# rohanpsingh/LearningHumanoidWalking

Hardware: AMD Instinct MI355X
Metric: env-steps/s (whole job): on-device rollout + GAE + PPO update (higher is better)
Workload: dtype f64 physics / f32 networks

## Files before the change

learninghumanoidwalking_amd/csrc/lhw_learner.h:

```cpp
#pragma once
#include "lhw_internal.h"

struct LearnerCore {
  int device = 0, D = 0, Dp = 0, A = 0, H = 0, learn_std = 0;
  float clip, ent_coeff, mirror_coeff, grad_clip, lr, adam_eps, beta1, beta2;
  int use_mirror = 0;
  size_t off_actor = 0, off_std = 0, off_critic = 0, n_critic = 0, n_params = 0;
  int *d_obs_src = nullptr, *d_act_src = nullptr;
  float *d_obs_sign = nullptr, *d_act_sign = nullptr;
  float *stats = nullptr;
  float *stats_part = nullptr;
  float *norm_part = nullptr;
  LhwDevMem mem;
};
#define SUMSQ_BLOCKS 128

int learner_check(const LhwPpoConfig* c, void** out, bool caps_ok);
void learner_init(LearnerCore& k, const LhwPpoConfig* c, size_t n_actor, size_t n_critic);
bool learner_mirror(LearnerCore& k, const LhwPpoConfig* c);
int learner_normalize(LearnerCore* k, const float* obs, int64_t R, const float* obs_mean, const float* obs_std, float* xn, float* xm, void* stream);
int learner_apply(LearnerCore* k, float* theta, float* grad, float* adam_m, float* adam_v, int64_t step, float grad_scale, void* stream);
int learner_grad_sqnorms(LearnerCore* k, float* out2_host);

struct AdamArgs {
  float *theta, *grad, *m, *v;
  size_t n0, off1, n1;
  int blocks0;
  float gscale;
  float* part;
  float* normsq_out;
  float max_norm, lr, beta1, beta2, eps, bc1, bc2sqrt;
};
AdamArgs learner_adam_args(const LearnerCore& k, float* theta, float* grad, float* adam_m, float* adam_v, int64_t step, float grad_scale);
__global__ void adam2_kernel(AdamArgs a);

struct StreamPair {
  hipStream_t s, sc;
  hipEvent_t ev_fork, ev_join;
  void fork() const { if (sc != s) { (void)hipEventRecord(ev_fork, s); (void)hipStreamWaitEvent(sc, ev_fork, 0); } }
  void join() const { if (sc != s) { (void)hipEventRecord(ev_join, sc); (void)hipStreamWaitEvent(s, ev_join, 0); } }
};

__global__ void normalize_kernel(const float* __restrict__ obs, int D, int Dp, size_t R, const float* __restrict__ mean, const float* __restrict__ stdv,
                                 float* __restrict__ xn, float* __restrict__ xm, const int* __restrict__ src, const float* __restrict__ sign);
__global__ void sample_kernel(const float* __restrict__ mu, int ldmu, int A, int N, const float* __restrict__ stdv, uint64_t seed, uint32_t env_base,
                              uint32_t counter, int deterministic, float* __restrict__ act, float* __restrict__ logp);
__global__ void ppo_loss_kernel(int B, int Rcap, int A, int Op, const float* __restrict__ ya, const float* __restrict__ yc, const float* __restrict__ act,
                                const float* __restrict__ old_logp, const float* __restrict__ adv, const float* __restrict__ ret,
                                const float* __restrict__ stdv, float clip, float mirror_coeff, int use_mirror, const int* __restrict__ act_src,
                                const float* __restrict__ act_sign, float* __restrict__ dya, float* __restrict__ dyc, float* __restrict__ dstd,
                                float* __restrict__ stats_part, const float* __restrict__ imit_target, const unsigned char* __restrict__ imit_mask,
                                float imit_coeff, float imit_inv_count, int seqB, float gscale);
__global__ void ppo_stats_rows_kernel(int B, int A, const float* __restrict__ rows, int ld, float imit_inv_count, float* __restrict__ stats_part);
__global__ void reduce_rows_kernel(const float* __restrict__ part, int nrows, int n, float* __restrict__ out);
__global__ void entropy_grad_kernel(const float* __restrict__ stdv, int A, float ent_coeff, float* __restrict__ grad_std);
```

learninghumanoidwalking_amd/csrc/lhw_learner.hip:

```cpp
#include "lhw_learner.h"

#include <cmath>
#include <mutex>
#include <vector>

#include "lhw_policy.h"
#include "lhw_rng.h"

__global__ void normalize_kernel(const float* __restrict__ obs, int D, int Dp, size_t R, const float* __restrict__ mean,
                                 const float* __restrict__ stdv, float* __restrict__ xn, float* __restrict__ xm,
                                 const int* __restrict__ src, const float* __restrict__ sign) {
  size_t i = (size_t)blockIdx.x * blockDim.x + threadIdx.x;
  if (i >= R * (size_t)Dp) return;
  size_t r = i / Dp;
  int j = (int)(i - r * Dp);
  float v = 0.f, vm = 0.f;
  if (j < D) {
    v = (obs[r * D + j] - mean[j]) / stdv[j];
    if (xm) vm = (sign[j] * obs[r * D + src[j]] - mean[j]) / stdv[j];
  }
  xn[i] = v;
  if (xm) xm[i] = vm;
}
__global__ void __launch_bounds__(256) sample_kernel(const float* __restrict__ mu, int ldmu, int A, int N, const float* __restrict__ stdv,
                                                     uint64_t seed, uint32_t env_base, uint32_t counter, int deterministic,
                                                     float* __restrict__ act, float* __restrict__ logp) {
  __shared__ float terms[8][32];
  LHW_LDS_POISON(terms);
  const int r = threadIdx.x >> 5, a = threadIdx.x & 31, n = blockIdx.x * 8 + r;
  if (n < N && a < A) {
    float term;
    act[(size_t)n * A + a] = lhw_policy_sample(mu[(size_t)n * ldmu + a], stdv[a], seed, env_base + n, counter, a, deterministic, &term);
    terms[r][a] = term;
  }
  __syncthreads();
  if (n < N && a == 0) {
    float lp = 0.f;
    for (int k = 0; k < A; k++) lp += terms[r][k];
    logp[n] = lp;
  }
}
__device__ __forceinline__ void ppo_stats_block(float (&vals)[NSTAT], float* __restrict__ stats_part) {
  __shared__ float red[NSTAT][4];
  LHW_LDS_POISON(red);
  for (int o = 32; o > 0; o >>= 1)
    for (int k = 0; k < NSTAT; k++) vals[k] += __shfl_xor(vals[k], o);
  int lane = threadIdx.x & 63, wave = threadIdx.x >> 6;
  if (lane == 0)
    for (int k = 0; k < NSTAT; k++) red[k][wave] = vals[k];
  __syncthreads();
  if (threadIdx.x < NSTAT) stats_part[(size_t)blockIdx.x * NSTAT + threadIdx.x] = (red[threadIdx.x][0] + red[threadIdx.x][1]) + (red[threadIdx.x][2] + red[threadIdx.x][3]);
}
__global__ void __launch_bounds__(256) ppo_loss_kernel(int B, int Rcap, int A, int Op, const float* __restrict__ ya,
                                                       const float* __restrict__ yc, const float* __restrict__ act,
                                                       const float* __restrict__ old_logp, const float* __restrict__ adv,
                                                       const float* __restrict__ ret, const float* __restrict__ stdv,
                                                       float clip, float mirror_coeff, int use_mirror,
                                                       const int* __restrict__ act_src, const float* __restrict__ act_sign,
                                                       float* __restrict__ dya, float* __restrict__ dyc,
                                                       float* __restrict__ dstd , float* __restrict__ stats_part,
                                                       const float* __restrict__ imit_target ,
                                                       const unsigned char* __restrict__ imit_mask , float imit_coeff,
                                                       float imit_inv_count, int seqB,
                                                       float gscale ) {
  int m = blockIdx.x * blockDim.x + threadIdx.x;
  size_t rn = (size_t)m, rm = (size_t)Rcap + m;
  if (seqB > 0 && use_mirror) { rn = (size_t)(m / seqB) * (2 * (size_t)seqB) + (size_t)(m % seqB); rm = rn + seqB; }
  const LhwPpoHead h{B, A, Op, act, old_logp, adv, ret, stdv, clip, mirror_coeff, use_mirror, act_src, act_sign, dstd, imit_target, imit_mask,
                     imit_coeff, imit_inv_count, gscale};
  float t[NSTAT] = {0, 0, 0, 0, 0, 0};
  const float invB = 1.f / (float)B, invBA = 1.f / ((float)B * (float)A);
  if (m < B) {
    lhw_ppo_actor_row(h, m, ya + rn * Op, ya + rm * Op, dya + rn * Op, dya + rm * Op, 1, t);
    float dv;
    t[1] = lhw_ppo_critic_row(h, m, yc[(size_t)m * 4], &dv);
    dyc[(size_t)m * 4] = dv;
    dyc[(size_t)m * 4 + 1] = 0.f; dyc[(size_t)m * 4 + 2] = 0.f; dyc[(size_t)m * 4 + 3] = 0.f;
  }
  float vals[NSTAT] = {t[0] * invB, t[1] * invB, t[2] * invBA, t[3] * invB, t[4] * invB, t[5] * imit_inv_count};
  ppo_stats_block(vals, stats_part);
}

__global__ void __launch_bounds__(256) ppo_stats_rows_kernel(int B, int A, const float* __restrict__ rows, int ld, float imit_inv_count,
                                                             float* __restrict__ stats_part) {
  const int m = blockIdx.x * blockDim.x + threadIdx.x;
  float t[NSTAT] = {0, 0, 0, 0, 0, 0};
  if (m < B)
    for (int k = 0; k < NSTAT; k++) t[k] = rows[(size_t)k * ld + m];
  const float invB = 1.f / (float)B, invBA = 1.f / ((float)B * (float)A);
  float vals[NSTAT] = {t[0] * invB, t[1] * invB, t[2] * invBA, t[3] * invB, t[4] * invB, t[5] * imit_inv_count};
  ppo_stats_block(vals, stats_part);
}

__global__ void reduce_rows_kernel(const float* __restrict__ part, int nrows, int n, float* __restrict__ out) {
  int k = threadIdx.x;
  if (k >= n) return;
  float s = 0.f;
  for (int b = 0; b < nrows; b++) s += part[(size_t)b * n + k];
  out[k] += s;
}

__global__ void entropy_grad_kernel(const float* __restrict__ stdv, int A, float ent_coeff, float* __restrict__ grad_std) {
  int a = threadIdx.x;
  if (a < A) grad_std[a] += -ent_coeff / ((float)A * stdv[a]);
}
__global__ void __launch_bounds__(256) sumsq2_kernel(const float* __restrict__ g0, size_t n0, const float* __restrict__ g1, size_t n1, float scale,
                                                     float* __restrict__ part ) {
  const int grp = blockIdx.x / SUMSQ_BLOCKS, b = blockIdx.x - grp * SUMSQ_BLOCKS;
  const float* __restrict__ g = grp ? g1 : g0;
  const size_t n = grp ? n1 : n0;
  float s = 0.f;
  for (size_t i = (size_t)b * blockDim.x + threadIdx.x; i < n; i += (size_t)SUMSQ_BLOCKS * blockDim.x) {
    float v = g[i] * scale;
    s += v * v;
  }
  for (int o = 32; o > 0; o >>= 1) s += __shfl_xor(s, o);
  __shared__ float red[4];
  LHW_LDS_POISON(red);
  if ((threadIdx.x & 63) == 0) red[threadIdx.x >> 6] = s;
  __syncthreads();
  if (threadIdx.x == 0) part[blockIdx.x] = (red[0] + red[1]) + (red[2] + red[3]);
}
__global__ void __launch_bounds__(256) adam2_kernel(AdamArgs a) {
  float *__restrict__ theta = a.theta, *__restrict__ grad = a.grad, *__restrict__ m = a.m, *__restrict__ v = a.v, *__restrict__ normsq_out = a.normsq_out;
  const float* __restrict__ part = a.part;
  const size_t n0 = a.n0, off1 = a.off1, n1 = a.n1;
  const int blocks0 = a.blocks0;
  const float gscale = a.gscale, max_norm = a.max_norm, lr = a.lr, beta1 = a.beta1, beta2 = a.beta2, eps = a.eps, bc1 = a.bc1, bc2sqrt = a.bc2sqrt;
  const int grp = (int)blockIdx.x >= blocks0 ? 1 : 0;
  __shared__ float nsq;
  LHW_LDS_POISON(nsq);
  if (threadIdx.x == 0) {
    float s = 0.f;
    for (int b = 0; b < SUMSQ_BLOCKS; b++) s += part[grp * SUMSQ_BLOCKS + b];
    nsq = s;
    if ((int)blockIdx.x == (grp ? blocks0 : 0)) normsq_out[grp] = s;
  }
  __syncthreads();
  const size_t i = (size_t)((int)blockIdx.x - (grp ? blocks0 : 0)) * blockDim.x + threadIdx.x;
  if (i >= (grp ? n1 : n0)) return;
  const size_t e = (grp ? off1 : 0) + i;
  float norm = sqrtf(nsq);
  float coef = max_norm / (norm + 1e-6f);
  coef = coef < 1.f ? coef : 1.f;
  float g = grad[e] * gscale * coef;
  float mi = beta1 * m[e] + (1.f - beta1) * g;
  float vi = beta2 * v[e] + (1.f - beta2) * g * g;
  m[e] = mi; v[e] = vi;
  float denom = sqrtf(vi) / bc2sqrt + eps;
  theta[e] -= (lr / bc1) * (mi / denom);
  grad[e] = 0.f;
}
__global__ void __launch_bounds__(256) gae_kernel(int T, int N, const float* __restrict__ rew, const float* __restrict__ val,
                                                  const uint8_t* __restrict__ done, const float* __restrict__ vterm,
                                                  const float* __restrict__ vfinal, double gamma, double lam,
                                                  float* __restrict__ ret, float* __restrict__ adv) {
  int n = blockIdx.x * blockDim.x + threadIdx.x;
  if (n >= N) return;
  double gae = 0.0, nextv = (double)vfinal[n];
  for (int t = T - 1; t >= 0; t--) {
    size_t i = (size_t)t * N + n;
    uint8_t f = done[i];
    if (f) {
      nextv = (f & 1) ? 0.0 : (double)vterm[i];
      gae = 0.0;
    }
    double v = (double)val[i];
    double delta = (double)rew[i] + gamma * nextv - v;
    gae = delta + gamma * lam * gae;
    double r = gae + v;
    ret[i] = (float)r;
    adv[i] = (float)r - val[i];
    nextv = v;
  }
}

#define MOM_BLOCKS 256
__global__ void __launch_bounds__(256) moments_kernel(const float* __restrict__ x, size_t n, double* __restrict__ part) {
  double s = 0, s2 = 0;
  for (size_t i = (size_t)blockIdx.x * blockDim.x + threadIdx.x; i < n; i += (size_t)gridDim.x * blockDim.x) {
    double v = x[i];
    s += v; s2 += v * v;
  }
  for (int o = 32; o > 0; o >>= 1) { s += __shfl_xor(s, o); s2 += __shfl_xor(s2, o); }
  __shared__ double red[2][4];
  LHW_LDS_POISON(red);
  if ((threadIdx.x & 63) == 0) { red[0][threadIdx.x >> 6] = s; red[1][threadIdx.x >> 6] = s2; }
  __syncthreads();
  if (threadIdx.x == 0) {
    part[2 * blockIdx.x] = (red[0][0] + red[0][1]) + (red[0][2] + red[0][3]);
    part[2 * blockIdx.x + 1] = (red[1][0] + red[1][1]) + (red[1][2] + red[1][3]);
  }
}
__global__ void moments_final_kernel(const double* __restrict__ part, int n, double* __restrict__ out) {
  if (threadIdx.x < 2) {
    double s = 0;
    for (int b = 0; b < n; b++) s += part[2 * b + threadIdx.x];
    out[threadIdx.x] = s;
  }
}
__global__ void scale_shift_kernel(float* __restrict__ x, size_t n, float mean, float inv) {
  size_t i = (size_t)blockIdx.x * blockDim.x + threadIdx.x;
  if (i < n) x[i] = (x[i] - mean) * inv;
}

__global__ void standardize_kernel(float* __restrict__ x, size_t n, const double* __restrict__ st, double eps) {
  const double cnt = st[2], mean = st[0] / cnt;
  const double var = fmax(0.0, (st[1] - cnt * mean * mean) / fmax(1.0, cnt - 1.0));
  const float mean_f = (float)mean, inv_f = (float)(1.0 / (sqrt(var) + eps));
  size_t i = (size_t)blockIdx.x * blockDim.x + threadIdx.x;
  if (i < n) x[i] = (x[i] - mean_f) * inv_f;
}
// ... 14 lines not shown
  k.use_mirror = c->mirror_obs_src != nullptr;
  k.off_actor = 0; k.off_std = n_actor; k.off_critic = k.off_std + pad4(k.A); k.n_critic = n_critic; k.n_params = k.off_critic + n_critic;
}
bool learner_mirror(LearnerCore& k, const LhwPpoConfig* c) {
  if (!k.use_mirror) return true;
  std::vector<int> osrc(k.Dp, 0), asrc(k.A, 0);
  std::vector<float> osgn(k.Dp, 0.f), asgn(k.A, 0.f);
  for (int j = 0; j < k.D; j++) { osrc[j] = c->mirror_obs_src[j]; osgn[j] = c->mirror_obs_sign[j]; if (osrc[j] < 0 || osrc[j] >= k.D) return false; }
  for (int j = 0; j < k.A; j++) { asrc[j] = c->mirror_act_src[j]; asgn[j] = c->mirror_act_sign[j]; if (asrc[j] < 0 || asrc[j] >= k.A) return false; }
  k.d_obs_src = k.mem.put(osrc.data(), osrc.size()); k.d_act_src = k.mem.put(asrc.data(), asrc.size());
  k.d_obs_sign = k.mem.put(osgn.data(), osgn.size()); k.d_act_sign = k.mem.put(asgn.data(), asgn.size());
  return !k.mem.failed();
}
int learner_normalize(LearnerCore* k, const float* obs, int64_t R, const float* obs_mean, const float* obs_std, float* xn, float* xm,
                             void* stream) {
  if (!k || !obs || !xn || R <= 0) return lhw_fail(LHW_ERR_ARG, "bad argument");
  if (xm && !k->use_mirror) return lhw_fail(LHW_ERR_ARG, "mirror output requested but no mirror tables configured");
  HIPCHK(hipSetDevice(k->device));
  size_t n = (size_t)R * k->Dp;
  hipLaunchKernelGGL(normalize_kernel, dim3((n + 255) / 256), dim3(256), 0, (hipStream_t)stream, obs, k->D, k->Dp, (size_t)R,
                     obs_mean, obs_std, xn, xm, k->d_obs_src, k->d_obs_sign);
  HIPCHK(hipGetLastError());
  return LHW_OK;
}
#define LHW_MAX_DEVICES 64
static int device_of(const void* ptr, int* dev) {
  hipPointerAttribute_t at;
  if (hipPointerGetAttributes(&at, ptr) != hipSuccess) return lhw_fail(LHW_ERR_ARG, "not a device pointer");
  if (at.device < 0 || at.device >= LHW_MAX_DEVICES) return lhw_fail(LHW_ERR_ARG, "device %d out of range", at.device);
  if (hipSetDevice(at.device) != hipSuccess) return lhw_fail(LHW_ERR_HIP, "hipSetDevice(%d) failed", at.device);
  *dev = at.device;
  return 0;
}

extern "C" int lhw_gae(int32_t T, int32_t N, const float* rew, const float* val, const uint8_t* done, const float* vterm,
                       const float* vfinal, double gamma, double lam, float* ret, float* adv, void* stream) {
  if (T <= 0 || N <= 0 || !rew || !val || !done || !vterm || !vfinal || !ret || !adv) return lhw_fail(LHW_ERR_ARG, "bad argument");
  int dev = 0;
  if (device_of(rew, &dev)) return LHW_ERR_HIP;
  hipLaunchKernelGGL(gae_kernel, dim3((N + 255) / 256), dim3(256), 0, (hipStream_t)stream, T, N, rew, val, done, vterm, vfinal,
                     gamma, lam, ret, adv);
  HIPCHK(hipGetLastError());
  return LHW_OK;
}

extern "C" int lhw_moments(const float* x, int64_t n, double* out2_dev, void* stream) {
  if (!x || !out2_dev || n <= 0) return lhw_fail(LHW_ERR_ARG, "bad argument");
  int dev = 0;
  if (device_of(x, &dev)) return LHW_ERR_HIP;
  static double* scratch_of[LHW_MAX_DEVICES] = {nullptr};
  static std::mutex mu;
  double* scratch;
  {
    std::lock_guard<std::mutex> lock(mu);
    if (!scratch_of[dev]) HIPCHK(lhw_malloc(&scratch_of[dev], sizeof(double) * 2 * MOM_BLOCKS));
    scratch = scratch_of[dev];
  }
  hipLaunchKernelGGL(moments_kernel, dim3(MOM_BLOCKS), dim3(256), 0, (hipStream_t)stream, x, (size_t)n, scratch);
  hipLaunchKernelGGL(moments_final_kernel, dim3(1), dim3(64), 0, (hipStream_t)stream, scratch, MOM_BLOCKS, out2_dev);
  HIPCHK(hipGetLastError());
  return LHW_OK;
}
extern "C" int lhw_scale_shift(float* x, int64_t n, float mean, float inv_scale, void* stream) {
  if (!x || n <= 0) return lhw_fail(LHW_ERR_ARG, "bad argument");
  int dev = 0;
  if (device_of(x, &dev)) return LHW_ERR_HIP;
  hipLaunchKernelGGL(scale_shift_kernel, dim3((n + 255) / 256), dim3(256), 0, (hipStream_t)stream, x, (size_t)n, mean, inv_scale);
  HIPCHK(hipGetLastError());
  return LHW_OK;
}

extern "C" int lhw_standardize(float* x, int64_t n, const double* stats3_dev, double eps, void* stream) {
  if (!x || !stats3_dev || n <= 0) return lhw_fail(LHW_ERR_ARG, "bad argument");
  int dev = 0;
  if (device_of(x, &dev)) return LHW_ERR_HIP;
  hipLaunchKernelGGL(standardize_kernel, dim3((n + 255) / 256), dim3(256), 0, (hipStream_t)stream, x, (size_t)n, stats3_dev, eps);
  HIPCHK(hipGetLastError());
  return LHW_OK;
}
AdamArgs learner_adam_args(const LearnerCore& k, float* theta, float* grad, float* adam_m, float* adam_v, int64_t step, float grad_scale) {
  const size_t na = k.learn_std ? k.off_std + k.A : k.off_std;
  const float bc1 = 1.f - powf(k.beta1, (float)step), bc2 = 1.f - powf(k.beta2, (float)step);
  return AdamArgs{theta, grad, adam_m, adam_v, na, k.off_critic, k.n_critic, (int)((na + 255) / 256), grad_scale, k.norm_part, k.stats + 8,
                  k.grad_clip, k.lr, k.beta1, k.beta2, k.adam_eps, bc1, sqrtf(bc2)};
}
static void clip_and_adam(const AdamArgs& a, hipStream_t s) {
  const int blocks1 = (int)((a.n1 + 255) / 256);
  hipLaunchKernelGGL(sumsq2_kernel, dim3(2 * SUMSQ_BLOCKS), dim3(256), 0, s, a.grad, a.n0, a.grad + a.off1, a.n1, a.gscale, a.part);
  hipLaunchKernelGGL(adam2_kernel, dim3(a.blocks0 + blocks1), dim3(256), 0, s, a);
}

int learner_apply(LearnerCore* k, float* theta, float* grad, float* adam_m, float* adam_v, int64_t step, float grad_scale, void* stream) {
  if (!k || !theta || !grad || !adam_m || !adam_v || step <= 0) return lhw_fail(LHW_ERR_ARG, "bad argument");
  HIPCHK(hipSetDevice(k->device));
  hipStream_t s = (hipStream_t)stream;
  clip_and_adam(learner_adam_args(*k, theta, grad, adam_m, adam_v, step, grad_scale), s);
  if (!k->learn_std) HIPCHK(hipMemsetAsync(grad + k->off_std, 0, sizeof(float) * pad4(k->A), s));
  HIPCHK(hipGetLastError());
  return LHW_OK;
}

int learner_grad_sqnorms(LearnerCore* k, float* out2_host) {
  if (!k || !out2_host) return lhw_fail(LHW_ERR_ARG, "null argument");
  HIPCHK(hipSetDevice(k->device));
  HIPCHK(hipDeviceSynchronize());
  HIPCHK(hipMemcpy(out2_host, k->stats + 8, 2 * sizeof(float), hipMemcpyDeviceToHost));
  return LHW_OK;
}
```

learninghumanoidwalking_amd/csrc/lhw_mlp_strip.hip:

```cpp
#include <hip/hip_runtime.h>

#include <cstdlib>

#include "../../include/lhw.h"
#include "lhw_internal.h"
#include "lhw_lstm_cell.h"
#include "lhw_lstm_steps.h"
#include "lhw_policy.h"

#ifndef __HIP_EMU__
typedef float f32x16 __attribute__((ext_vector_type(16)));
#endif

#define SH 256
#define SBK 16
#define SXK 64
#define SXW LHW_MLP_STRIP_MAX_IN_PAD
static_assert(SXK <= SH && SXW <= SH, "the input slab is a part of the activation slab");
static_assert(SXW == LHW_ROLLOUT_HISTORY_MAX_OBS_PAD, "every row the in-wave policy step of the history rollout takes has the strip update");
#define SKQ 32

template <int RT_, int CT_, int NW_>
struct StripShape {
  static constexpr int RT = RT_, CT = CT_, NW = NW_, ROWS = 32 * RT_, LD = ROWS + 4, THR = 64 * NW_;
// ... 245 lines not shown
  for (int q = 0; q < QW; q++)
#pragma unroll
    for (int i = 0; i < C::RT; i++)
#pragma unroll
      for (int r = 0; r < 16; r++) p[q][i][r] = 0.f;
#pragma unroll
  for (int q = 0; q < QW; q++) {
#pragma unroll 8
    for (int kk = 0; kk < SKQ / 2; kk++) {
      const int k = (wave * QW + q) * SKQ + kk * 2 + kh;
      const float bv = a.w3t[(size_t)k * a.Op + min(l31, a.O - 1)], b = l31 < a.O ? bv : 0.f;
#pragma unroll
      for (int i = 0; i < C::RT; i++) p[q][i] = __builtin_amdgcn_mfma_f32_32x32x2f32(L.S[k][32 * i + l31], b, p[q][i], 0, 0, 0);
    }
  }
  SCLK(10);
  __syncthreads();
  SCLK(11);
  float (*P)[C::ROWS][32] = reinterpret_cast<float (*)[C::ROWS][32]>(&L.S[0][0]);
#pragma unroll
  for (int q = 0; q < QW; q++)
#pragma unroll
    for (int i = 0; i < C::RT; i++)
#pragma unroll
      for (int r = 0; r < 16; r++) P[wave * QW + q][32 * i + (r & 3) + 8 * (r >> 2) + 4 * kh][l31] = p[q][i][r];
  __syncthreads();
  return P;
}

template <class C>
__device__ __forceinline__ float (*fwd_readout_chain(StripLds<C>& L, const MlpStripFwd& a))[C::ROWS][32] {
  static_assert(C::RT <= C::NW, "a wave per row tile");
  const int tid = threadIdx.x, lane = tid & 63, wave = tid >> 6;
  const int l31 = lane & 31, kh = lane >> 5;
  f32x16 p;
#pragma unroll
  for (int r = 0; r < 16; r++) p[r] = 0.f;
  if (wave < C::RT) {
#pragma unroll 8
    for (int kk = 0; kk < SH / 2; kk++) {
      const int k = kk * 2 + kh;
      const float bv = a.w3t[(size_t)k * a.Op + min(l31, a.O - 1)], b = l31 < a.O ? bv : 0.f;
      p = __builtin_amdgcn_mfma_f32_32x32x2f32(L.S[k][32 * wave + l31], b, p, 0, 0, 0);
    }
  }
  SCLK(10);
  __syncthreads();
  SCLK(11);
  float (*P)[C::ROWS][32] = reinterpret_cast<float (*)[C::ROWS][32]>(&L.S[0][0]);
  if (wave < C::RT) {
#pragma unroll
    for (int r = 0; r < 16; r++) P[0][32 * wave + (r & 3) + 8 * (r >> 2) + 4 * kh][l31] = p[r];
  }
  __syncthreads();
  return P;
}
template <int XK> struct ReadoutParts { static constexpr int N = XK > SXK ? 1 : SH / SKQ; };

template <class C, bool RB>
__device__ __forceinline__ void bwd_layers(StripLds<C>& L, WOp<C>& w, const float* __restrict__ w2, const float* __restrict__ w3, const int O,
                                           const SlabRows<C>& sr, const float* __restrict__ h1, const float* __restrict__ h2, float* __restrict__ dh2,
                                           float* __restrict__ dh1, const unsigned* __restrict__ bits1, const unsigned* __restrict__ bits2,
                                           unsigned (&rb1)[C::CT], unsigned (&rb2)[C::CT], const int c0) {
  float (*X)[C::LD] = &L.S[SH - SXK];
  SCLK(c0);
  f32x16 acc[C::RT][C::CT];
  zero_acc<C>(acc);
  slab_mma<C>(X, O, w3, SH, w, acc);
  wload<C>(w, w2, SH, SH, 0);
  SCLK(c0 + 1);
  __syncthreads();
  SCLK(c0 + 2);
  store_act<C, true, RB ? 2 : 0>(L, acc, nullptr, false, h2, dh2, sr, nullptr, bits2, rb2);
  SCLK(c0 + 3);
  __syncthreads();
  SCLK(c0 + 4);
  zero_acc<C>(acc);
  slab_mma<C>(L.S, SH, w2, SH, w, acc);
  SCLK(c0 + 5);
  store_act<C, false, RB ? 2 : 0>(L, acc, nullptr, false, h1, dh1, sr, nullptr, bits1, rb1);
  SCLK(c0 + 6);
}

template <class C, int XK>
__global__ void __launch_bounds__(C::THR, 2) mlp_fwd_strip_kernel(MlpStripFwd a) {
  __shared__ StripLds<C> L;
  LHW_LDS_POISON(L);
  const int tid = threadIdx.x;
  const int row0 = (int)blockIdx.x * C::ROWS;
  const SlabRows<C> sr = SlabRows<C>::consecutive(row0, a.R);
  unsigned rb1[C::CT], rb2[C::CT];
  fwd_hidden<C, false, XK>(L, a, sr, rb1, rb2);
  float (*P)[C::ROWS][32] = ReadoutParts<XK>::N == 1 ? fwd_readout_chain<C>(L, a) : fwd_readout_partials<C>(L, a);
  constexpr int NQ = ReadoutParts<XK>::N;
  for (int i = tid; i < C::ROWS * 32; i += C::THR) {
    const int row = i >> 5, col = i & 31;
    if (col < a.O && row0 + row < a.R) {
      float s = P[0][row][col];
#pragma unroll
      for (int q = 1; q < NQ; q++) s += P[q][row][col];
      s += a.b3[col];
      a.y[(size_t)(row0 + row) * a.Op + col] = s;
      if (a.act) {
        float term;
        a.act[(size_t)(row0 + row) * a.O + col] = lhw_policy_sample(s, a.stdv[col], a.seed, a.env_base + (unsigned)(row0 + row), a.counter, col, a.deterministic, &term);
        P[0][row][col] = term;
      }
    }
  }
  SCLK(12);
  if (a.act) {
    __syncthreads();
    for (int row = tid; row < C::ROWS; row += C::THR)
      if (row0 + row < a.R) {
        float lp = 0.f;
        for (int k = 0; k < a.O; k++) lp += P[0][row][k];
        a.logp[row0 + row] = lp;
      }
  }
}

template <class C>
__global__ void __launch_bounds__(C::THR, 2) mlp_bwd_strip_kernel(MlpStripBwd a) {
  __shared__ StripLds<C> L;
  LHW_LDS_POISON(L);
  const SlabRows<C> sr = SlabRows<C>::consecutive((int)blockIdx.x * C::ROWS, a.R);
  float (*X)[C::LD] = &L.S[SH - SXK];
  WOp<C> w;
  SCLK(0);
  wload<C>(w, a.w3, SH, a.O, 0);
  stage_input<C, SXK>(X, a.dy, a.Op, a.O, sr);
  __syncthreads();
  unsigned rb1[C::CT], rb2[C::CT];
  bwd_layers<C, false>(L, w, a.w2, a.w3, a.O, sr, a.h1, a.h2, a.dh2, a.dh1, a.bits1, a.bits2, rb1, rb2, 1);
}

template <class C, int CRITIC, int XK>
__global__ void __launch_bounds__(C::THR, 2) mlp_train_strip_kernel(MlpStripTrain t) {
  static_assert(C::RT == 2, "a twin slab is two row tiles");
  __shared__ StripLds<C> L;
  LHW_LDS_POISON(L);
  const MlpStripFwd& a = t.f;
  const int tid = threadIdx.x;
  const int nrow = t.twin0 > 0 ? 32 : C::ROWS;
  const SlabRows<C> sr = t.twin0 > 0 ? SlabRows<C>::twins((int)blockIdx.x * 32, a.R, t.twin0) : SlabRows<C>::consecutive((int)blockIdx.x * C::ROWS, a.R);
  unsigned rb1[C::CT], rb2[C::CT];
  fwd_hidden<C, true, XK>(L, a, sr, rb1, rb2);
  float (*P)[C::ROWS][32] = ReadoutParts<XK>::N == 1 ? fwd_readout_chain<C>(L, a) : fwd_readout_partials<C>(L, a);
  constexpr int NQ = ReadoutParts<XK>::N;
  for (int i = tid; i < C::ROWS * 32; i += C::THR) {
    const int row = i >> 5, col = i & 31;
    if (col < a.O) {
      float s = P[0][row][col];
#pragma unroll
      for (int q = 1; q < NQ; q++) s += P[q][row][col];
      s += a.b3[col];
      if (a.y && sr.live(row)) a.y[(size_t)sr.grow(row) * a.Op + col] = s;
      P[0][row][col] = s;
    }
  }
  SCLK(12);
  WOp<C> w;
  wload<C>(w, t.w3, SH, a.O, 0);
  __syncthreads();
  float (*X)[C::LD] = &L.S[SH - SXK];
  const int Kp = (a.O + SBK - 1) & ~(SBK - 1), Kz = max(Kp, a.Op);
  if (tid < nrow) {
    const int m = (int)blockIdx.x * nrow + tid;
    const bool twin = t.twin0 > 0;
    if (m < a.R) {
      if (CRITIC) {
        float dv;
        const float e2 = lhw_ppo_critic_row(t.head, m, P[0][tid][0], &dv);
        X[0][tid] = dv;
        for (int k = 1; k < Kz; k++) X[k][tid] = 0.f;
        t.stat_rows[(size_t)t.stat_ld + m] = e2;
      } else {
        float st[NSTAT];
        lhw_ppo_actor_row(t.head, m, &P[0][tid][0], twin ? &P[0][32 + tid][0] : nullptr, &X[0][tid], twin ? &X[0][32 + tid] : nullptr, C::LD, st);
        for (int k = a.Op; k < Kz; k++) { X[k][tid] = 0.f; if (twin) X[k][32 + tid] = 0.f; }
#pragma unroll
        for (int k = 0; k < NSTAT; k++)
          if (k != 1) t.stat_rows[(size_t)k * t.stat_ld + m] = st[k];
      }
    } else {
      for (int k = 0; k < Kz; k++) { X[k][tid] = 0.f; if (twin) X[k][32 + tid] = 0.f; }
    }
  }
  __syncthreads();
  SCLK(13);
  for (int i = tid; i < C::ROWS * a.Op; i += C::THR) {
    const int row = i / a.Op, k = i - row * a.Op;
    if (sr.live(row)) t.dy[(size_t)sr.grow(row) * a.Op + k] = X[k][row];
  }
  bwd_layers<C, true>(L, w, t.w2, t.w3, a.O, sr, nullptr, nullptr, t.dh2, t.dh1, nullptr, nullptr, rb1, rb2, 14);
}

template <int CRITIC>
__global__ void __launch_bounds__(256) ppo_head_rows_kernel(LhwPpoHead h, const float* y, int Op, int twin0, float* dy, float* stat_rows, int stat_ld) {
  const int m = (int)(blockIdx.x * blockDim.x + threadIdx.x);
  if (m >= h.B) return;
  if (CRITIC) {
    float dv;
    stat_rows[(size_t)stat_ld + m] = lhw_ppo_critic_row(h, m, y[(size_t)m * Op], &dv);
    dy[(size_t)m * Op] = dv;
    for (int k = 1; k < Op; k++) dy[(size_t)m * Op + k] = 0.f;
  } else {
    float st[NSTAT];
    lhw_ppo_actor_row(h, m, y + (size_t)m * Op, y + ((size_t)twin0 + m) * Op, dy + (size_t)m * Op, dy + ((size_t)twin0 + m) * Op, 1, st);
    for (int k = 0; k < NSTAT; k++)
      if (k != 1) stat_rows[(size_t)k * stat_ld + m] = st[k];
  }
}

struct TransposeJob { const float* W; float* WT; int rows, cols, ld, ldt, first; };
struct TransposeJobs { TransposeJob j[3]; };
__global__ void __launch_bounds__(256) transpose3_kernel(TransposeJobs J) {
  __shared__ float T[32][33];
  LHW_LDS_POISON(T);
  const int b = (int)blockIdx.x, m = b >= J.j[2].first ? 2 : (b >= J.j[1].first ? 1 : 0);
  const TransposeJob q = J.j[m];
  const int tx = threadIdx.x & 31, ty = threadIdx.x >> 5;
  const int tc = (q.cols + 31) / 32, t = b - q.first, r0 = (t / tc) * 32, c0 = (t % tc) * 32;
  for (int y = ty; y < 32; y += 8) T[y][tx] = (r0 + y < q.rows && c0 + tx < q.cols) ? q.W[(size_t)(r0 + y) * q.ld + c0 + tx] : 0.f;
  __syncthreads();
  for (int y = ty; y < 32; y += 8)
    if (c0 + y < q.cols && r0 + tx < q.rows) q.WT[(size_t)(c0 + y) * q.ldt + r0 + tx] = T[tx][y];
}

size_t mlp_strip_wt_floats(int Dp, int Op) { return (size_t)Dp * SH + (size_t)SH * SH + (size_t)SH * Op; }

void mlp_strip_prepare(const float* w1, const float* w2, const float* w3, int Dp, int O, int Op, float* wt, hipStream_t s) {
  float *w1t = wt, *w2t = wt + (size_t)Dp * SH, *w3t = w2t + (size_t)SH * SH;
  auto tiles = [](int rows, int cols) { return ((rows + 31) / 32) * ((cols + 31) / 32); };
  TransposeJobs J;
  J.j[0] = TransposeJob{w1, w1t, SH, Dp, Dp, SH, 0};
  J.j[1] = TransposeJob{w2, w2t, SH, SH, SH, SH, tiles(SH, Dp)};
  J.j[2] = TransposeJob{w3, w3t, O, SH, SH, Op, tiles(SH, Dp) + tiles(SH, SH)};
  hipLaunchKernelGGL(transpose3_kernel, dim3(J.j[2].first + tiles(O, SH)), dim3(256), 0, s, J);
}

void lhw_transpose3(const LhwTransposeJob (&jobs)[3], hipStream_t s) {
  TransposeJobs J;
  int first = 0;
  for (int m = 0; m < 3; m++) {
    J.j[m] = TransposeJob{jobs[m].W, jobs[m].WT, jobs[m].rows, jobs[m].cols, jobs[m].ld, jobs[m].ldt, first};
    first += ((jobs[m].rows + 31) / 32) * ((jobs[m].cols + 31) / 32);
  }
  if (first > 0) hipLaunchKernelGGL(transpose3_kernel, dim3(first), dim3(256), 0, s, J);
}

size_t mlp_strip_bits_words(size_t rows) { return (rows + StripBig::ROWS - 1) / StripBig::ROWS * StripBig::THR * StripBig::CT; }

bool mlp_strip_supported(int H, int Dp, int O, int Op) { return H == SH && Dp > 0 && Dp <= SXK && (Dp & 3) == 0 && O > 0 && O <= 32 && Op >= O; }
bool mlp_strip_wide_supported(int H, int Dp, int O, int Op) { return H == SH && Dp > SXK && Dp <= SXW && (Dp & 3) == 0 && O > 0 && O <= 32 && Op >= O; }

#define STRIP_SMALL_ROWS 16384
void mlp_strip_forward(const MlpStripFwd& a, hipStream_t s, int shape ) {
  if (a.R <= 0) return;
  const bool small = (shape == 1 || (shape == 0 && a.R <= STRIP_SMALL_ROWS)) && !a.bits1 && !a.bits2;
  const bool wide = a.Dp > SXK;
  const dim3 grid(small ? (a.R + StripSmall::ROWS - 1) / StripSmall::ROWS : (a.R + StripBig::ROWS - 1) / StripBig::ROWS), block(small ? StripSmall::THR : StripBig::THR);
  if (small && !wide) hipLaunchKernelGGL((mlp_fwd_strip_kernel<StripSmall, SXK>), grid, block, 0, s, a);
  else if (small) hipLaunchKernelGGL((mlp_fwd_strip_kernel<StripSmall, SXW>), grid, block, 0, s, a);
  else if (!wide) hipLaunchKernelGGL((mlp_fwd_strip_kernel<StripBig, SXK>), grid, block, 0, s, a);
  else hipLaunchKernelGGL((mlp_fwd_strip_kernel<StripBig, SXW>), grid, block, 0, s, a);
}

void mlp_strip_backward(const MlpStripBwd& a, hipStream_t s) {
  if (a.R <= 0) return;
  hipLaunchKernelGGL((mlp_bwd_strip_kernel<StripBig>), dim3((a.R + StripBig::ROWS - 1) / StripBig::ROWS), dim3(StripBig::THR), 0, s, a);
}

bool mlp_train_strip_supported(int H, int Dp, int O, int Op, int critic) {
  return mlp_strip_supported(H, Dp, O, Op) && Op <= SXK && (!critic || (O == 1 && Op == 4));
}
bool mlp_train_strip_wide_supported(int H, int Dp, int O, int Op, int critic) {
  return mlp_strip_wide_supported(H, Dp, O, Op) && Op <= SXK && (!critic || (O == 1 && Op == 4));
}

void mlp_train_strip(const MlpStripTrain& t, hipStream_t s) {
  if (t.f.R <= 0) return;
  const int nrow = t.twin0 > 0 ? 32 : StripBig::ROWS;
  const dim3 grid((t.f.R + nrow - 1) / nrow), block(StripBig::THR);
  const bool wide = t.f.Dp > SXK;
  if (t.critic && !wide) hipLaunchKernelGGL((mlp_train_strip_kernel<StripBig, 1, SXK>), grid, block, 0, s, t);
  else if (t.critic) hipLaunchKernelGGL((mlp_train_strip_kernel<StripBig, 1, SXW>), grid, block, 0, s, t);
// ... 694 lines not shown
```

learninghumanoidwalking_amd/csrc/lhw_ppo_head.h:

```cpp
#pragma once

#define NSTAT 6

struct LhwPpoHead {
  int B, A, Op;
  const float *act, *old_logp, *adv, *ret;
  const float* stdv;
  float clip, mirror_coeff;
  int use_mirror;
  const int* act_src;
  const float* act_sign;
  float* dstd;
  const float* imit_target;
  const unsigned char* imit_mask;
  float imit_coeff, imit_inv_count;
  float gscale;
};

__device__ __forceinline__ void lhw_ppo_actor_row(const LhwPpoHead& h, const int m, const float* mu_n, const float* mu_m, float* dmu_n,
                                                  float* dmu_m, const int ds, float* s) {
  const int A = h.A, Op = h.Op;
  const float* __restrict__ act = h.act;
  const float* __restrict__ stdv = h.stdv;
  const float invB = 1.f / (float)h.B, invBA = 1.f / ((float)h.B * (float)h.A);
  float s_mirror = 0, s_imit = 0;
  float lp = 0.f;
  for (int a = 0; a < A; a++) {
    float d = (act[(size_t)m * A + a] - mu_n[a]) / stdv[a];
    lp += -0.5f * d * d - logf(stdv[a]) - 0.9189385332046727f;
  }
  float logr = lp - h.old_logp[m];
  float ratio = expf(logr);
  float ad = h.adv[m];
  float cl = fminf(fmaxf(ratio, 1.f - h.clip), 1.f + h.clip);
  float cpi = ratio * ad, cll = cl * ad;
  s[0] = -fminf(cpi, cll);
  float dratio = (cpi <= cll) ? ad : 0.f;
  float dlp = -invB * dratio * ratio;
  s[3] = (ratio - 1.f) - logr;
  s[4] = fabsf(ratio - 1.f) > h.clip ? 1.f : 0.f;
  if (h.use_mirror) for (int a = 0; a < Op; a++) dmu_m[(size_t)a * ds] = 0.f;
  for (int a = 0; a < Op; a++) {
    float g = 0.f, gs = 0.f;
    if (a < A) {
      float mu = mu_n[a], sd = stdv[a], x = act[(size_t)m * A + a];
      g = dlp * (x - mu) / (sd * sd);
      gs = dlp * ((x - mu) * (x - mu) / (sd * sd * sd) - 1.f / sd);
      if (h.use_mirror) {
        float mm = h.act_sign[a] * mu_m[h.act_src[a]];
        float diff = mu - mm;
        s_mirror += diff * diff;
        g += h.mirror_coeff * 2.f * diff * invBA;
        dmu_m[(size_t)h.act_src[a] * ds] = -h.mirror_coeff * 2.f * diff * invBA * h.act_sign[a] * h.gscale;
      }
      if (h.imit_target && h.imit_mask[(size_t)m * A + a]) {
        float diff = mu - h.imit_target[(size_t)m * A + a];
        s_imit += diff * diff;
        g += h.imit_coeff * 2.f * diff * h.imit_inv_count;
      }
    }
    dmu_n[(size_t)a * ds] = g * h.gscale;
    if (h.dstd) h.dstd[(size_t)m * Op + a] = gs;
  }
  s[2] = s_mirror;
  s[5] = s_imit;
}

__device__ __forceinline__ float lhw_ppo_critic_row(const LhwPpoHead& h, const int m, const float v, float* dv) {
  const float invB = 1.f / (float)h.B;
  float e = h.ret[m] - v;
  *dv = -2.f * e * invB * h.gscale;
  return e * e;
}
```

Before: 4.152 million.

## Parallelize fused PPO head across threads and prefetch head inputs before readout

The actor PPO head inside the fused MLP strip kernel is split into per-element phases. Per-entry terms are computed by all threads into LDS scratch, then one thread per row reduces them, then all threads write the gradients. Head inputs (actions, std, old logp, advantage, returns) are prefetched into registers before the readout, and dy is written directly instead of in a separate copy pass. The separate memset that zeroes the std gradient is folded into the Adam kernel. The cost is more LDS scratch, extra syncthreads and more complex indexing.

```diff
diff --git a/learninghumanoidwalking_amd/csrc/lhw_learner.h b/learninghumanoidwalking_amd/csrc/lhw_learner.h
--- a/learninghumanoidwalking_amd/csrc/lhw_learner.h
+++ b/learninghumanoidwalking_amd/csrc/lhw_learner.h
@@ -30,6 +30,7 @@
   float* part;
   float* normsq_out;
   float max_norm, lr, beta1, beta2, eps, bc1, bc2sqrt;
+  size_t off_z; int nz;
 };
 AdamArgs learner_adam_args(const LearnerCore& k, float* theta, float* grad, float* adam_m, float* adam_v, int64_t step, float grad_scale);
 __global__ void adam2_kernel(AdamArgs a);
diff --git a/learninghumanoidwalking_amd/csrc/lhw_learner.hip b/learninghumanoidwalking_amd/csrc/lhw_learner.hip
--- a/learninghumanoidwalking_amd/csrc/lhw_learner.hip
+++ b/learninghumanoidwalking_amd/csrc/lhw_learner.hip
@@ -73,7 +73,7 @@
   if (m < B) {
     lhw_ppo_actor_row(h, m, ya + rn * Op, ya + rm * Op, dya + rn * Op, dya + rm * Op, 1, t);
     float dv;
-    t[1] = lhw_ppo_critic_row(h, m, yc[(size_t)m * 4], &dv);
+    t[1] = lhw_ppo_critic_row(h, ret[m], yc[(size_t)m * 4], &dv);
     dyc[(size_t)m * 4] = dv;
     dyc[(size_t)m * 4 + 1] = 0.f; dyc[(size_t)m * 4 + 2] = 0.f; dyc[(size_t)m * 4 + 3] = 0.f;
   }
@@ -128,6 +128,7 @@
   const int blocks0 = a.blocks0;
   const float gscale = a.gscale, max_norm = a.max_norm, lr = a.lr, beta1 = a.beta1, beta2 = a.beta2, eps = a.eps, bc1 = a.bc1, bc2sqrt = a.bc2sqrt;
   const int grp = (int)blockIdx.x >= blocks0 ? 1 : 0;
+  if (blockIdx.x == 0 && (int)threadIdx.x < a.nz) grad[a.off_z + threadIdx.x] = 0.f;
   __shared__ float nsq;
   LHW_LDS_POISON(nsq);
   if (threadIdx.x == 0) {
@@ -308,7 +309,7 @@
   const size_t na = k.learn_std ? k.off_std + k.A : k.off_std;
   const float bc1 = 1.f - powf(k.beta1, (float)step), bc2 = 1.f - powf(k.beta2, (float)step);
   return AdamArgs{theta, grad, adam_m, adam_v, na, k.off_critic, k.n_critic, (int)((na + 255) / 256), grad_scale, k.norm_part, k.stats + 8,
-                  k.grad_clip, k.lr, k.beta1, k.beta2, k.adam_eps, bc1, sqrtf(bc2)};
+                  k.grad_clip, k.lr, k.beta1, k.beta2, k.adam_eps, bc1, sqrtf(bc2), k.off_std, k.learn_std ? 0 : pad4(k.A)};
 }
 static void clip_and_adam(const AdamArgs& a, hipStream_t s) {
   const int blocks1 = (int)((a.n1 + 255) / 256);
@@ -321,7 +322,6 @@
   HIPCHK(hipSetDevice(k->device));
   hipStream_t s = (hipStream_t)stream;
   clip_and_adam(learner_adam_args(*k, theta, grad, adam_m, adam_v, step, grad_scale), s);
-  if (!k->learn_std) HIPCHK(hipMemsetAsync(grad + k->off_std, 0, sizeof(float) * pad4(k->A), s));
   HIPCHK(hipGetLastError());
   return LHW_OK;
 }
diff --git a/learninghumanoidwalking_amd/csrc/lhw_mlp_strip.hip b/learninghumanoidwalking_amd/csrc/lhw_mlp_strip.hip
--- a/learninghumanoidwalking_amd/csrc/lhw_mlp_strip.hip
+++ b/learninghumanoidwalking_amd/csrc/lhw_mlp_strip.hip
@@ -351,6 +351,14 @@
   SCLK(c0 + 6);
 }
 
+#define HEAD_PF 4
+template <class C>
+struct HeadLds {
+  static constexpr int LD = 33;
+  float x[C::ROWS * LD], d[C::ROWS * LD], dm[C::ROWS * LD], di[C::ROWS * LD], dlp[C::ROWS], log_sd[32];
+};
+static_assert(sizeof(float) * StripBig::ROWS * 32 + sizeof(HeadLds<StripBig>) <= sizeof(float) * (SH - SXK) * StripBig::LD, "P[0] and the head's scratch end below the dy slab");
+
 template <class C, int XK>
 __global__ void __launch_bounds__(C::THR, 2) mlp_fwd_strip_kernel(MlpStripFwd a) {
   __shared__ StripLds<C> L;
@@ -415,6 +423,22 @@
   const SlabRows<C> sr = t.twin0 > 0 ? SlabRows<C>::twins((int)blockIdx.x * 32, a.R, t.twin0) : SlabRows<C>::consecutive((int)blockIdx.x * C::ROWS, a.R);
   unsigned rb1[C::CT], rb2[C::CT];
   fwd_hidden<C, true, XK>(L, a, sr, rb1, rb2);
+  const LhwPpoHead& h = t.head;
+  const bool twin = t.twin0 > 0;
+  const int A = h.A, nE = nrow * a.Op, m0 = (int)blockIdx.x * nrow;
+  const float rOp = 1.f / (float)a.Op;
+  const int lsd = tid - (C::THR - 32);
+  float xpf[HEAD_PF], sdpf[HEAD_PF], olp = 0.f, adv = 0.f, ret = 0.f, sdl = 1.f;
+  if (!CRITIC) {
+#pragma unroll
+    for (int q = 0; q < HEAD_PF; q++) {
+      const int e = tid + q * C::THR, row = (int)(((float)e + 0.5f) * rOp), ac = e - row * a.Op;
+      xpf[q] = 0.f; sdpf[q] = 1.f;
+      if (e < nE && ac < A && m0 + row < a.R) { xpf[q] = h.act[(size_t)(m0 + row) * A + ac]; sdpf[q] = h.stdv[ac]; }
+    }
+    if (tid < nrow && m0 + tid < a.R) { olp = h.old_logp[m0 + tid]; adv = h.adv[m0 + tid]; }
+    if (lsd >= 0 && lsd < A) sdl = h.stdv[lsd];
+  } else if (tid < nrow && m0 + tid < a.R) ret = h.ret[m0 + tid];
   float (*P)[C::ROWS][32] = ReadoutParts<XK>::N == 1 ? fwd_readout_chain<C>(L, a) : fwd_readout_partials<C>(L, a);
   constexpr int NQ = ReadoutParts<XK>::N;
   for (int i = tid; i < C::ROWS * 32; i += C::THR) {
@@ -434,34 +458,89 @@
   __syncthreads();
   float (*X)[C::LD] = &L.S[SH - SXK];
   const int Kp = (a.O + SBK - 1) & ~(SBK - 1), Kz = max(Kp, a.Op);
-  if (tid < nrow) {
-    const int m = (int)blockIdx.x * nrow + tid;
-    const bool twin = t.twin0 > 0;
-    if (m < a.R) {
-      if (CRITIC) {
+  if (CRITIC) {
+    if (tid < nrow) {
+      const int m = m0 + tid;
+      if (m < a.R) {
         float dv;
-        const float e2 = lhw_ppo_critic_row(t.head, m, P[0][tid][0], &dv);
+        const float e2 = lhw_ppo_critic_row(h, ret, P[0][tid][0], &dv);
         X[0][tid] = dv;
         for (int k = 1; k < Kz; k++) X[k][tid] = 0.f;
+        for (int k = 0; k < a.Op; k++) t.dy[(size_t)m * a.Op + k] = k ? 0.f : dv;
         t.stat_rows[(size_t)t.stat_ld + m] = e2;
       } else {
-        float st[NSTAT];
-        lhw_ppo_actor_row(t.head, m, &P[0][tid][0], twin ? &P[0][32 + tid][0] : nullptr, &X[0][tid], twin ? &X[0][32 + tid] : nullptr, C::LD, st);
-        for (int k = a.Op; k < Kz; k++) { X[k][tid] = 0.f; if (twin) X[k][32 + tid] = 0.f; }
+        for (int k = 0; k < Kz; k++) X[k][tid] = 0.f;
+      }
+    }
+  } else {
+    HeadLds<C>& Hd = *reinterpret_cast<HeadLds<C>*>(&L.S[0][0] + C::ROWS * 32);
+    auto entry1 = [&](const int e, const float x, const float sd) {
+      const int row = (int)(((float)e + 0.5f) * rOp), ac = e - row * a.Op, m = m0 + row, o = row * HeadLds<C>::LD + ac;
+      if (ac < A && m < a.R) {
+        const float mu = P[0][row][ac];
+        Hd.x[o] = x;
+        Hd.d[o] = lhw_ppo_entry_d(x, mu, sd);
+        if (h.use_mirror) Hd.dm[o] = lhw_ppo_entry_mirror_diff(h, ac, mu, &P[0][32 + row][0]);
+        if (lhw_ppo_entry_imit(h, m, ac)) Hd.di[o] = lhw_ppo_entry_imit_diff(h, m, ac, mu);
+      }
+    };
+#pragma unroll
+    for (int q = 0; q < HEAD_PF; q++)
+      if (tid + q * C::THR < nE) entry1(tid + q * C::THR, xpf[q], sdpf[q]);
+    for (int e = tid + HEAD_PF * C::THR; e < nE; e += C::THR) {
+      const int row = (int)(((float)e + 0.5f) * rOp), ac = e - row * a.Op;
+      const bool on = ac < A && m0 + row < a.R;
+      entry1(e, on ? h.act[(size_t)(m0 + row) * A + ac] : 0.f, on ? h.stdv[ac] : 1.f);
+    }
+    if (lsd >= 0 && lsd < A) Hd.log_sd[lsd] = lhw_ppo_log_std(sdl);
+    __syncthreads();
+    if (tid < nrow) {
+      const int m = m0 + tid;
+      if (m < a.R) {
+        const float* hd = &Hd.d[tid * HeadLds<C>::LD];
+        float st[NSTAT], lp = 0.f, s_mirror = 0.f, s_imit = 0.f;
+        for (int ac = 0; ac < A; ac++) lhw_ppo_lp_term(lp, hd[ac], Hd.log_sd[ac]);
+        if (h.use_mirror)
+          for (int ac = 0; ac < A; ac++) lhw_ppo_sq_term(s_mirror, Hd.dm[tid * HeadLds<C>::LD + ac]);
+        if (h.imit_target)
+          for (int ac = 0; ac < A; ac++)
+            if (lhw_ppo_entry_imit(h, m, ac)) lhw_ppo_sq_term(s_imit, Hd.di[tid * HeadLds<C>::LD + ac]);
+        Hd.dlp[tid] = lhw_ppo_row_tail(h, lp, olp, adv, st);
+        st[2] = s_mirror;
+        st[5] = s_imit;
 #pragma unroll
         for (int k = 0; k < NSTAT; k++)
           if (k != 1) t.stat_rows[(size_t)k * t.stat_ld + m] = st[k];
       }
-    } else {
-      for (int k = 0; k < Kz; k++) { X[k][tid] = 0.f; if (twin) X[k][32 + tid] = 0.f; }
+    } else if (tid >= 64) {
+      for (int i = tid - 64; i < (Kz - a.Op) * C::ROWS; i += C::THR - 64) X[a.Op + i / C::ROWS][i % C::ROWS] = 0.f;
+    }
+    __syncthreads();
+    for (int e = tid; e < nE; e += C::THR) {
+      const int row = (int)(((float)e + 0.5f) * rOp), ac = e - row * a.Op, m = m0 + row, o = row * HeadLds<C>::LD + ac;
+      if (m < a.R) {
+        float dmu = 0.f, dsd = 0.f, dmm = 0.f;
+        int am = ac;
+        if (ac < A) {
+          const bool imit = lhw_ppo_entry_imit(h, m, ac);
+          lhw_ppo_entry_grad(h, ac, Hd.dlp[row], Hd.x[o], P[0][row][ac], h.stdv[ac], h.use_mirror ? Hd.dm[o] : 0.f, imit, imit ? Hd.di[o] : 0.f, &dmu, &dsd, &dmm);
+          if (twin) am = h.act_src[ac];
+        }
+        X[ac][row] = dmu;
+        t.dy[(size_t)m * a.Op + ac] = dmu;
+        if (h.dstd) h.dstd[(size_t)m * a.Op + ac] = dsd;
+        if (twin) {
+          X[am][32 + row] = dmm;
+          t.dy[((size_t)t.twin0 + m) * a.Op + am] = dmm;
+        }
+      } else {
+        X[ac][row] = 0.f;
+        if (twin) X[ac][32 + row] = 0.f;
+      }
     }
   }
   __syncthreads();
   SCLK(13);
-  for (int i = tid; i < C::ROWS * a.Op; i += C::THR) {
-    const int row = i / a.Op, k = i - row * a.Op;
-    if (sr.live(row)) t.dy[(size_t)sr.grow(row) * a.Op + k] = X[k][row];
-  }
   bwd_layers<C, true>(L, w, t.w2, t.w3, a.O, sr, nullptr, nullptr, t.dh2, t.dh1, nullptr, nullptr, rb1, rb2, 14);
 }
 
@@ -471,7 +550,7 @@
   if (m >= h.B) return;
   if (CRITIC) {
     float dv;
-    stat_rows[(size_t)stat_ld + m] = lhw_ppo_critic_row(h, m, y[(size_t)m * Op], &dv);
+    stat_rows[(size_t)stat_ld + m] = lhw_ppo_critic_row(h, h.ret[m], y[(size_t)m * Op], &dv);
     dy[(size_t)m * Op] = dv;
     for (int k = 1; k < Op; k++) dy[(size_t)m * Op + k] = 0.f;
   } else {
diff --git a/learninghumanoidwalking_amd/csrc/lhw_ppo_head.h b/learninghumanoidwalking_amd/csrc/lhw_ppo_head.h
--- a/learninghumanoidwalking_amd/csrc/lhw_ppo_head.h
+++ b/learninghumanoidwalking_amd/csrc/lhw_ppo_head.h
@@ -17,21 +17,22 @@
   float gscale;
 };
 
-__device__ __forceinline__ void lhw_ppo_actor_row(const LhwPpoHead& h, const int m, const float* mu_n, const float* mu_m, float* dmu_n,
-                                                  float* dmu_m, const int ds, float* s) {
-  const int A = h.A, Op = h.Op;
-  const float* __restrict__ act = h.act;
-  const float* __restrict__ stdv = h.stdv;
-  const float invB = 1.f / (float)h.B, invBA = 1.f / ((float)h.B * (float)h.A);
-  float s_mirror = 0, s_imit = 0;
-  float lp = 0.f;
-  for (int a = 0; a < A; a++) {
-    float d = (act[(size_t)m * A + a] - mu_n[a]) / stdv[a];
-    lp += -0.5f * d * d - logf(stdv[a]) - 0.9189385332046727f;
-  }
-  float logr = lp - h.old_logp[m];
+__device__ __forceinline__ float lhw_ppo_entry_d(const float x, const float mu, const float sd) { return (x - mu) / sd; }
+__device__ __forceinline__ float lhw_ppo_log_std(const float sd) { return logf(sd); }
+__device__ __forceinline__ void lhw_ppo_lp_term(float& lp, const float d, const float log_sd) { lp += -0.5f * d * d - log_sd - 0.9189385332046727f; }
+__device__ __forceinline__ void lhw_ppo_sq_term(float& s, const float diff) { s += diff * diff; }
+__device__ __forceinline__ float lhw_ppo_entry_mirror_diff(const LhwPpoHead& h, const int a, const float mu, const float* mu_m) {
+  float mm = h.act_sign[a] * mu_m[h.act_src[a]];
+  return mu - mm;
+}
+__device__ __forceinline__ bool lhw_ppo_entry_imit(const LhwPpoHead& h, const int m, const int a) { return h.imit_target && h.imit_mask[(size_t)m * h.A + a]; }
+__device__ __forceinline__ float lhw_ppo_entry_imit_diff(const LhwPpoHead& h, const int m, const int a, const float mu) {
+  return mu - h.imit_target[(size_t)m * h.A + a];
+}
+__device__ __forceinline__ float lhw_ppo_row_tail(const LhwPpoHead& h, const float lp, const float old_logp, const float ad, float* s) {
+  const float invB = 1.f / (float)h.B;
+  float logr = lp - old_logp;
   float ratio = expf(logr);
-  float ad = h.adv[m];
   float cl = fminf(fmaxf(ratio, 1.f - h.clip), 1.f + h.clip);
   float cpi = ratio * ad, cll = cl * ad;
   s[0] = -fminf(cpi, cll);
@@ -39,36 +40,66 @@
   float dlp = -invB * dratio * ratio;
   s[3] = (ratio - 1.f) - logr;
   s[4] = fabsf(ratio - 1.f) > h.clip ? 1.f : 0.f;
+  return dlp;
+}
+__device__ __forceinline__ void lhw_ppo_entry_grad(const LhwPpoHead& h, const int a, const float dlp, const float x, const float mu, const float sd,
+                                                   const float diff_mirror, const bool imit, const float diff_imit, float* dmu, float* dsd,
+                                                   float* dmu_m) {
+  const float invBA = 1.f / ((float)h.B * (float)h.A);
+  float g = dlp * (x - mu) / (sd * sd);
+  float gs = dlp * ((x - mu) * (x - mu) / (sd * sd * sd) - 1.f / sd);
+  if (h.use_mirror) {
+    float diff = diff_mirror;
+    g += h.mirror_coeff * 2.f * diff * invBA;
+    *dmu_m = -h.mirror_coeff * 2.f * diff * invBA * h.act_sign[a] * h.gscale;
+  }
+  if (imit) {
+    float diff = diff_imit;
+    g += h.imit_coeff * 2.f * diff * h.imit_inv_count;
+  }
+  *dmu = g * h.gscale;
+  *dsd = gs;
+}
+
+__device__ __forceinline__ void lhw_ppo_actor_row(const LhwPpoHead& h, const int m, const float* mu_n, const float* mu_m, float* dmu_n,
+                                                  float* dmu_m, const int ds, float* s) {
+  const int A = h.A, Op = h.Op;
+  const float* __restrict__ act = h.act;
+  const float* __restrict__ stdv = h.stdv;
+  float s_mirror = 0, s_imit = 0;
+  float lp = 0.f;
+  for (int a = 0; a < A; a++) {
+    float d = lhw_ppo_entry_d(act[(size_t)m * A + a], mu_n[a], stdv[a]);
+    lhw_ppo_lp_term(lp, d, lhw_ppo_log_std(stdv[a]));
+  }
+  const float dlp = lhw_ppo_row_tail(h, lp, h.old_logp[m], h.adv[m], s);
   if (h.use_mirror) for (int a = 0; a < Op; a++) dmu_m[(size_t)a * ds] = 0.f;
   for (int a = 0; a < Op; a++) {
     float g = 0.f, gs = 0.f;
     if (a < A) {
-      float mu = mu_n[a], sd = stdv[a], x = act[(size_t)m * A + a];
-      g = dlp * (x - mu) / (sd * sd);
-      gs = dlp * ((x - mu) * (x - mu) / (sd * sd * sd) - 1.f / sd);
+      float mu = mu_n[a], diff_mirror = 0.f, diff_imit = 0.f, gm = 0.f;
       if (h.use_mirror) {
-        float mm = h.act_sign[a] * mu_m[h.act_src[a]];
-        float diff = mu - mm;
-        s_mirror += diff * diff;
-        g += h.mirror_coeff * 2.f * diff * invBA;
-        dmu_m[(size_t)h.act_src[a] * ds] = -h.mirror_coeff * 2.f * diff * invBA * h.act_sign[a] * h.gscale;
+        diff_mirror = lhw_ppo_entry_mirror_diff(h, a, mu, mu_m);
+        lhw_ppo_sq_term(s_mirror, diff_mirror);
       }
-      if (h.imit_target && h.imit_mask[(size_t)m * A + a]) {
-        float diff = mu - h.imit_target[(size_t)m * A + a];
-        s_imit += diff * diff;
-        g += h.imit_coeff * 2.f * diff * h.imit_inv_count;
+      const bool imit = lhw_ppo_entry_imit(h, m, a);
+      if (imit) {
+        diff_imit = lhw_ppo_entry_imit_diff(h, m, a, mu);
+        lhw_ppo_sq_term(s_imit, diff_imit);
       }
+      lhw_ppo_entry_grad(h, a, dlp, act[(size_t)m * A + a], mu, stdv[a], diff_mirror, imit, diff_imit, &g, &gs, &gm);
+      if (h.use_mirror) dmu_m[(size_t)h.act_src[a] * ds] = gm;
     }
-    dmu_n[(size_t)a * ds] = g * h.gscale;
+    dmu_n[(size_t)a * ds] = g;
     if (h.dstd) h.dstd[(size_t)m * Op + a] = gs;
   }
   s[2] = s_mirror;
   s[5] = s_imit;
 }
 
-__device__ __forceinline__ float lhw_ppo_critic_row(const LhwPpoHead& h, const int m, const float v, float* dv) {
+__device__ __forceinline__ float lhw_ppo_critic_row(const LhwPpoHead& h, const float ret, const float v, float* dv) {
   const float invB = 1.f / (float)h.B;
-  float e = h.ret[m] - v;
+  float e = ret - v;
   *dv = -2.f * e * invB * h.gscale;
   return e * e;
 }
```

New measurement: 4.184 million, median of 6. No clear change (+0.8%).
